# Darioxavierl/OFDM-LTE

Measured on AMD Instinct MI355X. Metric: LTE subframes/sec (20 MHz, 64-QAM, Rayleigh+turbo) at 1/2/4/8 GPU; BER match, higher is better.
Workload: dtype f64

## Files before the change

ofdm-lte_amd/csrc/lte_turbo.hip:

```cpp
#include "lte_common.h"
#include "lte_internal.h"
#include "lte_dev.h"

namespace lte {


constexpr int DM_CH = 64;
#ifndef LTE_DM_NT
#define LTE_DM_NT 0
#endif
template <class R>
__device__ __forceinline__ void dm_store(R* dst, R v, bool add) {
  if (add) *dst = *dst + (R)0.5 * v;
  else if (LTE_DM_NT & 1) __builtin_nontemporal_store((R)0.5 * ((R)0 + v), dst);
  else *dst = (R)0.5 * ((R)0 + v);
}

template <class R>
__global__ __launch_bounds__(256) void k_dematch(const R* __restrict__ llr, int T, int B,
                                                 const int32_t* __restrict__ rx_map, int add,
                                                 R* const* __restrict__ blk, const int64_t* __restrict__ rows,
                                                 int ch, int g0) {
  __shared__ R tile[64][DM_CH + 1];
  const int g = g0 + blockIdx.y;
  const int t0 = blockIdx.x * DM_CH;
  const int nt = min(DM_CH, T - t0);
  const int c4 = (threadIdx.x & 15) * 4;
  for (int f = threadIdx.x >> 4; f < 64; f += 16) {
    const int b = g * 64 + f;
    const R* src = llr + (size_t)b * T + t0;
    R v[4] = {(R)0, (R)0, (R)0, (R)0};
    if (b < B) {
#pragma unroll
      for (int e = 0; e < 4; ++e)
        if (c4 + e < nt) v[e] = src[c4 + e];
    }
#pragma unroll
    for (int e = 0; e < 4; ++e) tile[f][c4 + e] = v[e];
  }
  __syncthreads();
  const int wv = __builtin_amdgcn_readfirstlane(threadIdx.x >> 6), f = threadIdx.x & 63;
  for (int c = wv; c < nt; c += 4) {
    const int m = rx_map[t0 + c];
    if (m < 0) continue;
    const int r = m >> 24, row = m & 0xFFFFFF;
    dm_store(&blk[r][turbo_elem_ch(ch, rows[r], g, row) + f], tile[f][c], add != 0);
  }
}

template <class R>
int launch_dematch(hipStream_t s, const R* llr, int T, int B, const int32_t* rx_map, int n_layers, R* const* blk,
                   const int64_t* rows, int ch, int g0, int add0) {
  const int G = (B + 63) / 64 - g0;
  if (G < 1 || G > 65535 || n_layers < 1) return (int)hipErrorInvalidValue;
  for (int k = 0; k < n_layers; ++k) {
    hipLaunchKernelGGL(k_dematch<R>, dim3((T + DM_CH - 1) / DM_CH, G), dim3(256), 0, s, llr, T, B,
                       rx_map + (size_t)k * T, k > 0 || add0 ? 1 : 0, blk, rows, ch, g0);
    const int e = (int)hipGetLastError();
    if (e) return e;
  }
  return 0;
}

#ifndef LTE_DZ_RE64
#define LTE_DZ_RE64 8
#endif
template <class R> constexpr int dz_re() { return sizeof(R) == 8 ? LTE_DZ_RE64 : 16; }
template <class R, int BPS>
__global__ __launch_bounds__(256) void k_dematch_zn(const cx<R>* __restrict__ z, const R* __restrict__ nv, int n_re,
                                                    int nd, int n_nv, int nv_grp, int nv_sh, int B,
                                                    const int32_t* __restrict__ rx_map, int add,
                                                    R* const* __restrict__ blk, const int64_t* __restrict__ rows,
                                                    int ch, int g0) {
  using V = cx<R>;
  constexpr int DZ_RE = dz_re<R>(), TC = DZ_RE * BPS, PER = 64 * DZ_RE / 256;
  __shared__ R tile[64][TC + 1];
  const int g = g0 + blockIdx.y;
  const int re0 = blockIdx.x * DZ_RE;
  const int nr = min(DZ_RE, n_re - re0);
  V zv[PER];
  R nvv[PER];
#pragma unroll
  for (int k = 0; k < PER; ++k) {
    const int e = threadIdx.x + k * 256, f = e / DZ_RE, r = e % DZ_RE, b = g * 64 + f;
    const bool ok = b < B && r < nr;
    const size_t i = (size_t)b * n_re + re0 + r;
    const int l = (re0 + r) / nd, j = re0 + r - l * nd;
    if (LTE_DM_NT & 2) {
      zv[k] = ok ? mkc(__builtin_nontemporal_load(&z[i].x), __builtin_nontemporal_load(&z[i].y)) : mkc((R)0, (R)0);
      nvv[k] = ok ? __builtin_nontemporal_load(&nv[(size_t)b * n_nv + (l / nv_grp) * (nd >> nv_sh) + (j >> nv_sh)])
                  : (R)1;
    } else {
      zv[k] = ok ? z[i] : mkc((R)0, (R)0);
      nvv[k] = ok ? nv[(size_t)b * n_nv + (l / nv_grp) * (nd >> nv_sh) + (j >> nv_sh)] : (R)1;
    }
  }
#pragma unroll
  for (int k = 0; k < PER; ++k) {
    const int e = threadIdx.x + k * 256, f = e / DZ_RE, r = e % DZ_RE;
    R o[BPS];
    soft_demap<BPS>(zv[k], nvv[k], o);
#pragma unroll
    for (int m = 0; m < BPS; ++m) tile[f][r * BPS + m] = o[m];
  }
  __syncthreads();
  const int t0 = re0 * BPS, nt = nr * BPS;
  const int wv = __builtin_amdgcn_readfirstlane(threadIdx.x >> 6), f = threadIdx.x & 63;
  for (int c = wv; c < nt; c += 4) {
    const int m = rx_map[t0 + c];
    if (m < 0) continue;
    const int r = m >> 24, row = m & 0xFFFFFF;
    dm_store(&blk[r][turbo_elem_ch(ch, rows[r], g, row) + f], tile[f][c], add != 0);
  }
}

template <class R>
int launch_dematch_zn(hipStream_t s, const cx<R>* z, const R* nv, int n_re, int nd, int bps, int B,
                      const int32_t* rx_map, int n_layers, R* const* blk, const int64_t* rows, int ch, int g0,
                      int nv_pairs, int add0) {
  const int G = (B + 63) / 64 - g0;
  if (G < 1 || G > 65535 || (bps != 4 && bps != 6) || n_layers < 1 || nd < 1) return (int)hipErrorInvalidValue;
  if (nv_pairs && (nd & 1)) return (int)hipErrorInvalidValue;
  const int nv_grp = nv_pairs ? 1 : 14, nv_sh = nv_pairs ? 1 : 0;
  const int n_nv = ((n_re / nd + nv_grp - 1) / nv_grp) * (nd >> nv_sh);
  constexpr int DZ = dz_re<R>();
  const dim3 grid((n_re + DZ - 1) / DZ, G);
  const int T = n_re * bps;
  for (int k = 0; k < n_layers; ++k) {
    const int32_t* mp = rx_map + (size_t)k * T;
    if (bps == 4)
      hipLaunchKernelGGL((k_dematch_zn<R, 4>), grid, dim3(256), 0, s, z, nv, n_re, nd, n_nv, nv_grp, nv_sh, B, mp,
                         k > 0 || add0 ? 1 : 0, blk, rows, ch, g0);
    else
      hipLaunchKernelGGL((k_dematch_zn<R, 6>), grid, dim3(256), 0, s, z, nv, n_re, nd, n_nv, nv_grp, nv_sh, B, mp,
                         k > 0 || add0 ? 1 : 0, blk, rows, ch, g0);
    const int e = (int)hipGetLastError();
    if (e) return e;
  }
  return 0;
}

template int launch_dematch<float>(hipStream_t, const float*, int, int, const int32_t*, int, float* const*,
                                   const int64_t*, int, int, int);
template int launch_dematch<double>(hipStream_t, const double*, int, int, const int32_t*, int, double* const*,
                                    const int64_t*, int, int, int);
template int launch_dematch_zn<float>(hipStream_t, const float2*, const float*, int, int, int, int, const int32_t*,
                                      int, float* const*, const int64_t*, int, int, int, int);
template int launch_dematch_zn<double>(hipStream_t, const double2*, const double*, int, int, int, int,
                                       const int32_t*, int, double* const*, const int64_t*, int, int, int, int);


template <class R>
__global__ __launch_bounds__(256) void k_harq_zero(const int32_t* __restrict__ zmap, int nz,
                                                   R* const* __restrict__ blk, const int64_t* __restrict__ rows,
                                                   int ch) {
  const int i = blockIdx.x * 4 + __builtin_amdgcn_readfirstlane(threadIdx.x >> 6);
  if (i >= nz) return;
  const int m = zmap[i], r = m >> 24, row = m & 0xFFFFFF;
  blk[r][turbo_elem_ch(ch, rows[r], blockIdx.y, row) + (threadIdx.x & 63)] = (R)0;
}

template <class R>
int launch_harq_zero(hipStream_t s, const int32_t* zmap, int nz, int G, R* const* blk, const int64_t* rows, int ch) {
  if (nz < 1 || G < 1 || G > 65535) return (int)hipErrorInvalidValue;
  hipLaunchKernelGGL(k_harq_zero<R>, dim3((nz + 3) / 4, G), dim3(256), 0, s, zmap, nz, blk, rows, ch);
  return (int)hipGetLastError();
}
template int launch_harq_zero<float>(hipStream_t, const int32_t*, int, int, float* const*, const int64_t*, int);
template int launch_harq_zero<double>(hipStream_t, const int32_t*, int, int, double* const*, const int64_t*, int);

__global__ __launch_bounds__(64) void k_harq_latch(int B, int t, uint32_t* __restrict__ frame_err,
                                                   uint32_t* __restrict__ frame_crc, uint32_t* __restrict__ tx_used,
                                                   uint32_t* __restrict__ l_err, uint32_t* __restrict__ l_crc,
                                                   uint32_t* __restrict__ skip) {
  const int g = blockIdx.x, b = g * 64 + (int)threadIdx.x;
  bool active = false;
  if (b < B) {
    if (t == 0 || !l_crc[b]) {
      const uint32_t e = frame_err[b], c = frame_crc[b];
      tx_used[b] = (uint32_t)(t + 1);
      l_err[b] = e;
      l_crc[b] = c;
      active = c == 0;
    } else {
      frame_err[b] = l_err[b];
      frame_crc[b] = l_crc[b];
    }
  }
  const unsigned long long still = __ballot(active);
  if (threadIdx.x == 0) skip[g] = still == 0ull ? 1u : 0u;
}

int launch_harq_latch(hipStream_t s, int B, int t, uint32_t* frame_err, uint32_t* frame_crc, uint32_t* tx_used,
                      uint32_t* l_err, uint32_t* l_crc, uint32_t* skip) {
  if (B < 1 || t < 0) return (int)hipErrorInvalidValue;
  hipLaunchKernelGGL(k_harq_latch, dim3((B + 63) / 64), dim3(64), 0, s, B, t, frame_err, frame_crc, tx_used, l_err,
                     l_crc, skip);
  return (int)hipGetLastError();
}

__global__ __launch_bounds__(256) void k_rate_dematch(const double* __restrict__ llr, int E, int Ncb, int n_out,
                                                      const int32_t* __restrict__ src0, int64_t ncb,
                                                      double* __restrict__ out) {
  const int64_t t = (int64_t)blockIdx.x * 256 + threadIdx.x;
  if (t >= ncb * n_out) return;
  const int64_t c = t / n_out;
  const int j = (int)(t - c * n_out);
  double v = 0.0;
  const double* l = llr + c * E;
  for (int i = src0[j]; i >= 0 && i < E; i += Ncb) v = v + l[i];
  out[t] = v;
}

int launch_rate_dematch(hipStream_t s, const double* llr, int E, int Ncb, int n_out, const int32_t* src0, int64_t ncb,
                        double* out) {
  const int64_t n = ncb * n_out;
  if (n <= 0) return 0;
  hipLaunchKernelGGL(k_rate_dematch, dim3((unsigned)((n + 255) / 256)), dim3(256), 0, s, llr, E, Ncb, n_out, src0, ncb,
                     out);
  return (int)hipGetLastError();
}

struct BitWriter {
  uint32_t* p;
  uint64_t acc;
  int n;
  __device__ __forceinline__ void put(uint32_t bits, int nb) {
    acc = (acc << nb) | (nb == 32 ? (uint64_t)bits : (uint64_t)(bits & ((1u << nb) - 1u)));
    n += nb;
    if (n >= 32) {
      *p++ = (uint32_t)(acc >> (n - 32));
      n -= 32;
    }
  }
  __device__ __forceinline__ void flush() {
    if (n) *p = (uint32_t)(acc << (32 - n));
  }
};


__device__ __forceinline__ uint32_t rsc_word(uint32_t u, int nb, uint32_t& s0, uint32_t& s1, uint32_t& s2,
                                             uint32_t* fw) {
  uint32_t y = u ^ (u >> 2) ^ (u >> 3) ^ (u >> 4);
  y ^= y >> 7;
  y ^= y >> 14;
  y ^= y >> 28;
  const uint32_t a = y ^ (s0 ? 0x72e5cb97u : 0u) ^ (s1 ? 0xe5cb972eu : 0u) ^ (s2 ? 0xb972e5cbu : 0u);
  const uint32_t q = a ^ ((a >> 1) | (s0 << 31)) ^ ((a >> 3) | (s2 << 31) | (s1 << 30) | (s0 << 29));
  s0 = (a >> (32 - nb)) & 1u;
  s1 = (a >> (33 - nb)) & 1u;
  s2 = (a >> (34 - nb)) & 1u;
  *fw = a;
  return q;
}

__device__ __forceinline__ uint32_t rsc_tail(uint32_t& s0, uint32_t& s1, uint32_t& s2) {
  const uint32_t fb = 0u, par = fb ^ s0 ^ s2;
  s2 = s1; s1 = s0; s0 = fb;
  return fb | (par << 1);
}

constexpr int ENC_SEG = 4;
constexpr int ENC_MAXSW = 48;
constexpr int ENC_CH = 16;

struct X2Tab { uint32_t v[16]; };
constexpr X2Tab make_x2tab(uint32_t poly) {
  X2Tab t{};
  uint32_t b = 2u;
  for (int j = 0; j < 16; ++j) {
    t.v[j] = b;
    uint32_t r = 0u;
    for (int i = 23; i >= 0; --i) {
      r = ((r << 1) & 0xFFFFFFu) ^ ((r & 0x800000u) ? poly : 0u);
      r ^= ((b >> i) & 1u) ? b : 0u;
    }
    b = r;
  }
  return t;
}
__constant__ X2Tab kX2B = make_x2tab((uint32_t)CRC24B_POLY);

__device__ __forceinline__ uint32_t crcb_xpow(int e) {
  uint32_t r = 1u;
  for (int j = 0; j < 16; ++j)
    if ((e >> j) & 1) r = gf24_mul(r, kX2B.v[j], (uint32_t)CRC24B_POLY);
  return r;
}

__device__ __forceinline__ uint32_t rsc_zero_steps(uint32_t st, int n) {
  uint32_t s0 = st & 1u, s1 = (st >> 1) & 1u, s2 = (st >> 2) & 1u;
  for (int k = n % 7; k > 0; --k) {
    const uint32_t fb = s1 ^ s2;
    s2 = s1; s1 = s0; s0 = fb;
  }
  return s0 | (s1 << 1) | (s2 << 2);
}

__device__ __forceinline__ uint32_t rsc_seg_start(const uint32_t* fin, int q, int lane, int K, int SW) {
  uint32_t st = 0u;
  for (int p = 0; p < q; ++p) {
    const int len = max(0, min(K, 32 * (p + 1) * SW) - 32 * p * SW);
    st = rsc_zero_steps(st, len) ^ fin[p * 64 + lane];
  }
  return st;
}

__global__ __launch_bounds__(64 * ENC_SEG) void k_encode(const uint32_t* __restrict__ pw, int PW, int KWmax,
                                                         uint32_t* __restrict__ enc, int EW,
                                                         const CbInfo* __restrict__ cbi, int B,
                                                         const uint16_t* __restrict__ qmask, int qstride) {
  extern __shared__ uint32_t esm[];
  uint32_t* cwl = esm;
  uint32_t* xch = esm + (size_t)KWmax * 64;
  __shared__ uint32_t crc_t[256];
  for (int i = threadIdx.x; i < 256; i += blockDim.x) crc_t[i] = crc24_table_entry(i, (uint32_t)CRC24B_POLY);
  const int G = (B + 63) >> 6;
  const int r = blockIdx.x / G;
  const int lane = threadIdx.x & 63, q = __builtin_amdgcn_readfirstlane(threadIdx.x >> 6);
  const int b = (blockIdx.x - r * G) * 64 + lane;
  const bool act = b < B;
  const CbInfo ci = cbi[r];
  const int K = ci.K, F = ci.F, C = gridDim.x / G;
  const int KW = (K + 31) >> 5, KWf = K >> 5;
  const int SW = (KW + ENC_SEG - 1) / ENC_SEG;
  const int w0 = min(KW, q * SW), w1 = min(KW, w0 + SW);
  const bool last = w0 < w1 && w1 == KW;
  const uint32_t* tb = pw + (size_t)(act ? b : 0) * PW;
  uint32_t* e = enc + ((size_t)(act ? b : 0) * C + r) * 3 * EW;
  const int Kd = ci.crc ? K - 24 : K;
  const int64_t base = (int64_t)ci.off - F;
  const int64_t i00 = base >> 5;
  const int o = (int)(base & 31);
  auto ldw = [&](int64_t i) -> uint32_t { return (i >= 0 && i < PW) ? tb[i] : 0u; };
  __syncthreads();
  uint32_t crc = 0u;
  {
    uint32_t wa = ldw(i00 + w0), wb = ldw(i00 + w0 + 1);
    for (int w = w0; w < w1; ++w) {
      const uint32_t wn = ldw(i00 + w + 2);
      const int p0 = w * 32;
      uint32_t t = o ? ((wa << o) | (wb >> (32 - o))) : wa;
      if (p0 < F) t &= (F - p0 >= 32) ? 0u : (0xFFFFFFFFu >> (F - p0));
      const int db = min(32, max(0, Kd - p0));
      t &= db >= 32 ? 0xFFFFFFFFu : ~(0xFFFFFFFFu >> db);
      if (ci.crc)
#pragma unroll
        for (int k = 0; k < 4; ++k)
          if (8 * k < db) crc = ((crc << 8) & 0xFFFFFFu) ^ crc_t[((crc >> 16) ^ (t >> (24 - 8 * k))) & 0xFFu];
      cwl[w * 64 + lane] = t;
      wa = wb;
      wb = wn;
    }
  }
  xch[q * 64 + lane] = (ci.crc && 32 * w0 < Kd)
                           ? gf24_mul(crc, crcb_xpow(Kd - min(32 * w1, Kd)), (uint32_t)CRC24B_POLY) : 0u;
  __syncthreads();
  if (ci.crc) {
    crc = 0u;
#pragma unroll
    for (int p = 0; p < ENC_SEG; ++p) crc ^= xch[p * 64 + lane];
    const uint32_t L = crc << 8;
    for (int w = max(w0, Kd >> 5); w < w1; ++w) {
      const int p0 = 32 * w;
      cwl[w * 64 + lane] |= p0 <= Kd ? (L >> (Kd - p0)) : (L << (p0 - Kd));
    }
  }
  uint32_t s0 = 0u, s1 = 0u, s2 = 0u, f;
  uint32_t F2 = 0u;
  const uint16_t* qm = qmask + (size_t)r * qstride;
  for (int w = w0; w < w1; ++w) {
    const uint32_t cwv = cwl[w * 64 + lane];
    const int nb = min(32, K - 32 * w);
    (void)rsc_word(cwv, nb, s0, s1, s2, &f);
    const uint32_t* qw = reinterpret_cast<const uint32_t*>(qm + 32 * w);
#pragma unroll
    for (int j = 0; j < 32; j += 2) {
      const uint32_t pr = qw[j >> 1];
      F2 ^= (pr & 0xFFFFu) & (0u - ((cwv >> (31 - j)) & 1u));
      F2 ^= (pr >> 16) & (0u - ((cwv >> (30 - j)) & 1u));
    }
  }
  xch[(ENC_SEG + q) * 64 + lane] = s0 | (s1 << 1) | (s2 << 2);
  xch[(2 * ENC_SEG + q) * 64 + lane] = F2;
  __syncthreads();
  uint32_t st = rsc_seg_start(xch + ENC_SEG * 64, q, lane, K, SW);
  s0 = st & 1u; s1 = (st >> 1) & 1u; s2 = (st >> 2) & 1u;
  uint32_t pf = 0, pq = 0;
  int pnb = 0;
  for (int wc = w0; wc < w1; wc += ENC_CH) {
    uint32_t fb[ENC_CH], qb[ENC_CH];
#pragma unroll
    for (int j = 0; j < ENC_CH; ++j) {
      const int w = wc + j;
      fb[j] = qb[j] = 0u;
      if (w >= w1) continue;
      const int nb = min(32, K - 32 * w);
      const uint32_t qq = rsc_word(cwl[w * 64 + lane], nb, s0, s1, s2, &f);
      if (nb == 32) { fb[j] = f; qb[j] = qq; }
      else { pf = f; pq = qq; pnb = nb; }
    }
    if (act) {
#pragma unroll
      for (int j = 0; j < ENC_CH; ++j)
        if (wc + j < min(w1, KWf)) e[wc + j] = fb[j];
#pragma unroll
      for (int j = 0; j < ENC_CH; ++j)
        if (wc + j < min(w1, KWf)) e[EW + wc + j] = qb[j];
    }
  }
  if (last && act) {
    BitWriter wr0{e + KWf, 0, 0}, wr1{e + EW + KWf, 0, 0};
    if (pnb) {
      wr0.put(pf >> (32 - pnb), pnb);
      wr1.put(pq >> (32 - pnb), pnb);
    }
    for (int t = 0; t < 3; ++t) {
      const uint32_t v = rsc_tail(s0, s1, s2);
      wr0.put(v & 1u, 1);
      wr1.put(v >> 1, 1);
    }
    wr0.flush();
    wr1.flush();
  }
  {
    uint32_t fall = 0u;
#pragma unroll
    for (int p = 0; p < ENC_SEG; ++p) fall ^= xch[(2 * ENC_SEG + p) * 64 + lane];
    uint32_t st2 = 0u;
    for (int t = 0; t < q; ++t) {
      const int len = max(0, min(K, 32 * (t + 1) * SW) - 32 * t * SW);
      st2 = rsc_zero_steps(st2, len) ^ ((fall >> (3 * t)) & 7u);
    }
    s0 = st2 & 1u; s1 = (st2 >> 1) & 1u; s2 = (st2 >> 2) & 1u;
  }
  pq = 0;
  pnb = 0;
  {
    const int k0 = 32 * w0;
    int pi0 = (int)(((int64_t)ci.f1 * k0 + (int64_t)ci.f2 * k0 % K * k0) % K);
    int d0 = (int)(((int64_t)ci.f1 + (int64_t)ci.f2 * (2 * (int64_t)k0 + 1)) % K);
    const float invK = 1.0f / (float)K;
    const int f2l = (int)(((int64_t)ci.f2 * lane * (lane - 1)) % K);
    const char* cwb = reinterpret_cast<const char*>(cwl) + 4 * lane;
    for (int w = w0; w < w1; w += 2) {
      int x = pi0 + (int)((lane * (int64_t)d0) % K) + f2l;
      x -= (int)((float)x * invK) * K;
      x += x < 0 ? K : 0;
      x -= x >= K ? K : 0;
      const int rowb = (x >> 5) << 8, shf = x & 31;
      uint32_t qw[2] = {0u, 0u};
#pragma unroll
      for (int h = 0; h < 2; ++h) {
        if (w + h >= w1) break;
        const int nb = min(32, K - 32 * (w + h));
        uint32_t u = 0u;
#pragma unroll
        for (int j = 0; j < 32; ++j) {
          const int a = __builtin_amdgcn_readlane(rowb, 32 * h + j);
          const int sh = __builtin_amdgcn_readlane(shf, 32 * h + j);
          const uint32_t v = *reinterpret_cast<const uint32_t*>(cwb + a);
          u |= ((v << sh) >> 31) << (31 - j);
        }
        const uint32_t qq = rsc_word(u, nb, s0, s1, s2, &f);
        if (nb == 32) qw[h] = qq;
        else { pq = qq; pnb = nb; }
      }
      if (act) {
        if (w < KWf) e[2 * EW + w] = qw[0];
        if (w + 1 < min(w1, KWf)) e[2 * EW + w + 1] = qw[1];
      }
      pi0 = (int)(((int64_t)pi0 + 64 * (int64_t)d0 + (int64_t)ci.f2 * 64 * 63) % K);
      d0 = (int)(((int64_t)d0 + 128 * (int64_t)ci.f2) % K);
    }
  }
  if (last && act) {
    BitWriter wr2{e + 2 * EW + KWf, 0, 0};
    if (pnb) wr2.put(pq >> (32 - pnb), pnb);
    for (int t = 0; t < 3; ++t) {
      const uint32_t v = rsc_tail(s0, s1, s2);
      const int pos = K + 3 + t;
      if (v & 1u) e[pos >> 5] |= 1u << (31 - (pos & 31));
      wr2.put(v >> 1, 1);
    }
    wr2.flush();
  }
}

void encode_qmask(const CbInfo* cbs, int C, int qstride, uint16_t* out) {
  std::fill(out, out + (size_t)C * qstride, (uint16_t)0);
  for (int r = 0; r < C; ++r) {
    const int K = cbs[r].K, KW = (K + 31) / 32, SW = (KW + ENC_SEG - 1) / ENC_SEG;
    uint16_t v[7];
    uint32_t st = 1u;
    for (int m = 0; m < 7; ++m) {
      v[m] = (uint16_t)st;
      const uint32_t s0 = st & 1u, s1 = (st >> 1) & 1u, s2 = (st >> 2) & 1u;
      st = (s1 ^ s2) | (s0 << 1) | (s1 << 2);
    }
    for (int64_t k = 0; k < K; ++k) {
      const int p = (int)((cbs[r].f1 * k + (int64_t)cbs[r].f2 * k % K * k) % K);
      const int t = (int)(k / (32 * SW)), end = std::min(32 * SW * (t + 1), K);
      out[(size_t)r * qstride + p] = (uint16_t)(v[(end - 1 - k) % 7] << (3 * t));
    }
  }
}

int launch_encode(hipStream_t s, const uint32_t* pw, int PW, int KWmax, uint32_t* enc, int EW,
                  const CbInfo* cbi_dev, int C, int B, const uint16_t* qmask, int qstride) {
  const int64_t blocks = (int64_t)C * ((B + 63) / 64);
  const size_t shm = ((size_t)KWmax * 64 + 3 * ENC_SEG * 64) * sizeof(uint32_t);
  if (blocks > 0x7FFFFFFF || KWmax > 4 * ENC_MAXSW + 1 || shm > 65536 || !qmask) return (int)hipErrorInvalidValue;
  hipLaunchKernelGGL(k_encode, dim3((unsigned)blocks), dim3(64 * ENC_SEG), shm, s, pw, PW, KWmax, enc, EW, cbi_dev,
                     B, qmask, qstride);
  return (int)hipGetLastError();
}


__device__ __forceinline__ uint32_t get32s(const uint32_t* w, int64_t st, int64_t p, int64_t nwords) {
  const int64_t i = p >> 5;
  const int o = (int)(p & 31);
  const uint32_t a = w[i * st];
  if (o == 0) return a;
  const uint32_t b = (i + 1 < nwords) ? w[(i + 1) * st] : 0u;
  return (a << o) | (b >> (32 - o));
}

constexpr int CRC_SEG = 8;
constexpr int CRC_MAXC = 32;
struct CrcSeg { uint32_t x[CRC_SEG]; };

__global__ __launch_bounds__(64 * CRC_SEG) void k_crc_count(const CbInfo* __restrict__ cbi, int C,
                                                            uint32_t* const* __restrict__ dec,
                                                            const int* __restrict__ KW, int B,
                                                            const uint32_t* __restrict__ pw, int PW, int n_bits,
                                                            int SW, CrcSeg xs, uint32_t* __restrict__ frame_err,
                                                            uint32_t* __restrict__ frame_crc,
                                                            uint8_t* __restrict__ cap_bits, int b0,
                                                            const uint64_t* __restrict__ fid, uint64_t seed) {
  __shared__ uint32_t T[1024];
  __shared__ uint32_t part[3][CRC_SEG][64];
  __shared__ int s_off[CRC_MAXC], s_end[CRC_MAXC], s_F[CRC_MAXC], s_kw[CRC_MAXC];
  __shared__ const uint32_t* s_dec[CRC_MAXC];
  crc24_slice4_fill(T, (uint32_t)CRC24A_POLY);
  if (threadIdx.x < C) {
    const CbInfo ci = cbi[threadIdx.x];
    s_off[threadIdx.x] = ci.off;
    s_end[threadIdx.x] = ci.off + ci.info;
    s_F[threadIdx.x] = ci.F;
    s_kw[threadIdx.x] = KW[threadIdx.x];
    s_dec[threadIdx.x] = dec[threadIdx.x];
  }
  __syncthreads();
  const int lane = threadIdx.x & 63, seg = __builtin_amdgcn_readfirstlane(threadIdx.x >> 6);
  const int b = b0 + blockIdx.x * 64 + lane;
  const bool act = b < B;
  const int bb = act ? b : b0;
  const int g = bb >> 6, gl = bb & 63;
  const uint32_t* tx = pw + (size_t)bb * PW;
  const uint64_t fr = fid ? fid[bb] : 0ull;
  u32x4 rv{0u, 0u, 0u, 0u};
  int rvg = -1;
  const int Btb = n_bits + 24;
  const int nw = (Btb + 31) >> 5;
  const int w0 = seg * SW, w1 = min(nw, w0 + SW);
  uint32_t crc = 0, err = 0, rx_crc = 0;
  int r = 0, off = s_off[0], end = s_end[0], F = s_F[0], kw = s_kw[0];
  const uint32_t* base = s_dec[0] + (size_t)g * kw * 64 + gl;
  for (int w = w0; w < w1; ++w) {
    uint32_t word = 0;
    int got = 0;
    const int want = min(32, Btb - 32 * w);
    while (got < want) {
      const int j = 32 * w + got;
      while (j >= end) {
        ++r;
        off = s_off[r]; end = s_end[r]; F = s_F[r]; kw = s_kw[r];
        base = s_dec[r] + (size_t)g * kw * 64 + gl;
      }
      const int avail = min(want - got, end - j);
      const uint32_t v = get32s(base, 64, (int64_t)F + (j - off), kw);
      const uint32_t m = avail >= 32 ? 0xFFFFFFFFu : ~(0xFFFFFFFFu >> avail);
      word |= (v & m) >> got;
      got += avail;
    }
    const int dbits = min(32, max(0, n_bits - 32 * w));
    if (dbits == 32) {
      crc = crc24_slice4(T, crc, word);
    } else {
      int k = 0;
      for (; k + 8 <= dbits; k += 8) {
        const uint32_t byte = (word >> (24 - k)) & 0xFFu;
        crc = ((crc << 8) & 0xFFFFFFu) ^ T[((crc >> 16) ^ byte) & 0xFFu];
      }
      for (; k < dbits; ++k) {
        const uint32_t bit = (word >> (31 - k)) & 1u;
        const uint32_t msb = (crc >> 23) & 1u;
        crc = (crc << 1) & 0xFFFFFFu;
        if (msb ^ bit) crc ^= (uint32_t)CRC24A_POLY;
      }
      for (int q = max(0, n_bits - 32 * w); q < want; ++q)
        rx_crc |= ((word >> (31 - q)) & 1u) << (23 - (32 * w + q - n_bits));
    }
    if (dbits > 0) {
      const uint32_t m = dbits >= 32 ? 0xFFFFFFFFu : ~(0xFFFFFFFFu >> dbits);
      uint32_t t;
      if (fid) {
        if ((w >> 2) != rvg) {
          rvg = w >> 2;
          rv = rng4(seed, fr, RNG_STREAM_BITS, (uint32_t)rvg);
        }
        t = (w & 3) == 0 ? rv.x : (w & 3) == 1 ? rv.y : (w & 3) == 2 ? rv.z : rv.w;
      } else {
        t = tx[w];
      }
      err += __popc((word ^ t) & m);
    }
    if (cap_bits && act) {
      for (int q = 0; q < dbits; ++q) cap_bits[(size_t)b * n_bits + 32 * w + q] = (word >> (31 - q)) & 1u;
    }
  }
  part[0][seg][lane] = gf24_mul(crc, xs.x[seg], (uint32_t)CRC24A_POLY);
  part[1][seg][lane] = err;
  part[2][seg][lane] = rx_crc;
  __syncthreads();
  if (seg == 0 && act) {
    uint32_t c = 0, e = 0, rc = 0;
#pragma unroll
    for (int s2 = 0; s2 < CRC_SEG; ++s2) {
      c ^= part[0][s2][lane];
      e += part[1][s2][lane];
      rc |= part[2][s2][lane];
    }
    frame_err[b] = e;
    frame_crc[b] = (c == rc) ? 1u : 0u;
  }
}

int launch_crc_count(hipStream_t s, const CbInfo* cbi_dev, int C, uint32_t* const* dec, const int* KW, int B,
                     const uint32_t* pw, int PW, int n_bits, uint32_t* frame_err, uint32_t* frame_crc,
                     uint8_t* cap_bits, int b0, const uint64_t* fid, uint64_t seed) {
  if (b0 < 0 || b0 >= B || n_bits < 0 || C < 1 || C > CRC_MAXC) return (int)hipErrorInvalidValue;
  const int nw = (n_bits + 24 + 31) >> 5;
  const int SW = (nw + CRC_SEG - 1) / CRC_SEG;
  CrcSeg xs{};
  for (int sg = 0; sg < CRC_SEG; ++sg) {
    const int end = std::min(32 * (sg + 1) * SW, n_bits);
    xs.x[sg] = gf24_xpow((uint64_t)(n_bits - std::max(end, 0)), (uint32_t)CRC24A_POLY);
  }
  hipLaunchKernelGGL(k_crc_count, dim3((B - b0 + 63) / 64), dim3(64 * CRC_SEG), 0, s, cbi_dev, C, dec, KW, B, pw, PW,
                     n_bits, SW, xs, frame_err, frame_crc, cap_bits, b0, fid, seed);
  return (int)hipGetLastError();
}

}
```

Measured before the change: 180,000.

## Restructure dematch_zn to loop over OFDM symbols with prefetch and grouped blocks

Replaces the per-RE-tile soft-demap and dematch kernel with one whose blocks own a subcarrier chunk and loop over all symbols. The next symbol's z, noise-variance, map and row pointers are prefetched while the current tile is written out. Destination addresses are computed once per tile column and broadcast with readlane, and the add/store path and channel count become template parameters. Block indices are grouped by 64-row batches to improve locality. This cuts launch-grid size, repeated index maths and load latency, at the cost of a serial symbol loop per block, fewer blocks, and higher register use.

```diff
diff --git a/ofdm-lte_amd/csrc/lte_turbo.hip b/ofdm-lte_amd/csrc/lte_turbo.hip
--- a/ofdm-lte_amd/csrc/lte_turbo.hip
+++ b/ofdm-lte_amd/csrc/lte_turbo.hip
@@ -66,6 +66,10 @@
 #define LTE_DZ_RE64 8
 #endif
 template <class R> constexpr int dz_re() { return sizeof(R) == 8 ? LTE_DZ_RE64 : 16; }
+#ifndef LTE_DZ_ORDER
+#define LTE_DZ_ORDER 2
+#endif
+#if LTE_DZ_ORDER == 0
 template <class R, int BPS>
 __global__ __launch_bounds__(256) void k_dematch_zn(const cx<R>* __restrict__ z, const R* __restrict__ nv, int n_re,
                                                     int nd, int n_nv, int nv_grp, int nv_sh, int B,
@@ -139,6 +143,158 @@
   }
   return 0;
 }
+#else
+constexpr int DZ_GW = LTE_DZ_ORDER == 2 ? 8 : 32;
+
+template <class R, bool ADD>
+__device__ __forceinline__ void dz_store(__attribute__((address_space(1))) R* dst, R old, R v) {
+  if (ADD) *dst = old + (R)0.5 * v;
+  else if (LTE_DM_NT & 1) __builtin_nontemporal_store((R)0.5 * ((R)0 + v), dst);
+  else *dst = (R)0.5 * ((R)0 + v);
+}
+
+template <class R, int BPS, int CH, bool ADD>
+__global__ __launch_bounds__(256) void k_dematch_zn(const cx<R>* __restrict__ z, const R* __restrict__ nv, int n_sym,
+                                                    int nd, int n_nv, int nv_grp, int nv_sh, int B,
+                                                    const int32_t* __restrict__ rx_map, R* const* __restrict__ blk,
+                                                    const int64_t* __restrict__ rows, int G, int g0) {
+  using V = cx<R>;
+  using GP = __attribute__((address_space(1))) R*;
+  constexpr int DZ_RE = dz_re<R>(), TC = DZ_RE * BPS, PER = 64 * DZ_RE / 256, NI = TC / 4;
+  static_assert(TC % 4 == 0 && NI <= 64, "one lane per tile column of a wave");
+  __shared__ R tile[64][TC + 1];
+  const int nj = (nd + DZ_RE - 1) / DZ_RE;
+  const int q = blockIdx.x / (DZ_GW * nj), id = blockIdx.x - q * DZ_GW * nj, w = min(DZ_GW, G - q * DZ_GW);
+  const int g = g0 + q * DZ_GW + id % w, j0 = (id / w) * DZ_RE;
+  const int nr = min(DZ_RE, nd - j0), nt = nr * BPS, n_re = n_sym * nd;
+  const int wv = __builtin_amdgcn_readfirstlane(threadIdx.x >> 6), lane = threadIdx.x & 63;
+  const int c = wv + 4 * lane;
+  const bool mok = lane < NI && c < nt;
+  const int32_t* mp = rx_map + (size_t)j0 * BPS + c;
+  auto ld_map = [&](int l) -> int { return mok && l < n_sym ? mp[(size_t)l * nd * BPS] : -1; };
+  int m1 = ld_map(0), m2 = ld_map(1);
+  size_t zi[PER], ni[PER];
+  bool ok[PER];
+#pragma unroll
+  for (int k = 0; k < PER; ++k) {
+    const int e = threadIdx.x + k * 256, f = e / DZ_RE, r = e % DZ_RE, b = g * 64 + f;
+    ok[k] = b < B && r < nr;
+    zi[k] = (size_t)b * n_re + j0 + r;
+    ni[k] = (size_t)b * n_nv + ((j0 + r) >> nv_sh);
+  }
+  V zv[PER];
+  R nvv[PER];
+  auto ld_z = [&](int l) {
+#pragma unroll
+    for (int k = 0; k < PER; ++k) {
+      const size_t i = zi[k] + (size_t)l * nd;
+      if (LTE_DM_NT & 2)
+        zv[k] = ok[k] ? mkc(__builtin_nontemporal_load(&z[i].x), __builtin_nontemporal_load(&z[i].y))
+                      : mkc((R)0, (R)0);
+      else
+        zv[k] = ok[k] ? z[i] : mkc((R)0, (R)0);
+    }
+  };
+  auto ld_nv = [&](int l) {
+#pragma unroll
+    for (int k = 0; k < PER; ++k) {
+      const size_t i = ni[k] + (size_t)(l / nv_grp) * (nd >> nv_sh);
+      if (LTE_DM_NT & 2) nvv[k] = ok[k] ? __builtin_nontemporal_load(&nv[i]) : (R)1;
+      else nvv[k] = ok[k] ? nv[i] : (R)1;
+    }
+  };
+  R* rb = nullptr;
+  int64_t rr = 0;
+  auto ld_row = [&]() {
+    if (m1 >= 0) {
+      rb = blk[m1 >> 24];
+      rr = rows[m1 >> 24];
+    }
+  };
+  ld_z(0);
+  ld_nv(0);
+  ld_row();
+  for (int l = 0; l < n_sym; ++l) {
+    const uint64_t dst = m1 >= 0 ? (uint64_t)(rb + turbo_elem<CH>(rr, g, m1 & 0xFFFFFF)) : 0;
+#pragma unroll
+    for (int k = 0; k < PER; ++k) {
+      const int e = threadIdx.x + k * 256, f = e / DZ_RE, r = e % DZ_RE;
+      R o[BPS];
+      soft_demap<BPS>(zv[k], nvv[k], o);
+#pragma unroll
+      for (int m = 0; m < BPS; ++m) tile[f][r * BPS + m] = o[m];
+    }
+    __syncthreads();
+    m1 = m2;
+    if (l + 1 < n_sym) {
+      ld_z(l + 1);
+      if ((l + 1) % nv_grp == 0) ld_nv(l + 1);
+      ld_row();
+      m2 = ld_map(l + 2);
+    }
+    R v[NI], old[NI];
+    GP d[NI];
+#pragma unroll
+    for (int i = 0; i < NI; ++i) {
+      v[i] = tile[lane][wv + 4 * i];
+      const uint32_t lo = __builtin_amdgcn_readlane((int)(uint32_t)dst, i);
+      const uint32_t hi = __builtin_amdgcn_readlane((int)(uint32_t)(dst >> 32), i);
+      d[i] = (GP)(((uint64_t)hi << 32) | lo);
+    }
+    if (ADD) {
+#pragma unroll
+      for (int i = 0; i < NI; ++i) old[i] = d[i] ? d[i][lane] : (R)0;
+    }
+#pragma unroll
+    for (int i = 0; i < NI; ++i)
+      if (d[i]) dz_store<R, ADD>(d[i] + lane, old[i], v[i]);
+    __syncthreads();
+  }
+}
+
+template <class R, int BPS, int CH>
+static void dz_launch(hipStream_t s, int nblk, const cx<R>* z, const R* nv, int n_sym, int nd, int n_nv, int nv_grp,
+                      int nv_sh, int B, const int32_t* mp, bool add, R* const* blk, const int64_t* rows, int G,
+                      int g0) {
+  if (add)
+    hipLaunchKernelGGL((k_dematch_zn<R, BPS, CH, true>), dim3(nblk), dim3(256), 0, s, z, nv, n_sym, nd, n_nv, nv_grp,
+                       nv_sh, B, mp, blk, rows, G, g0);
+  else
+    hipLaunchKernelGGL((k_dematch_zn<R, BPS, CH, false>), dim3(nblk), dim3(256), 0, s, z, nv, n_sym, nd, n_nv, nv_grp,
+                       nv_sh, B, mp, blk, rows, G, g0);
+}
+
+template <class R>
+int launch_dematch_zn(hipStream_t s, const cx<R>* z, const R* nv, int n_re, int nd, int bps, int B,
+                      const int32_t* rx_map, int n_layers, R* const* blk, const int64_t* rows, int ch, int g0,
+                      int nv_pairs, int add0) {
+  const int G = (B + 63) / 64 - g0;
+  if (G < 1 || G > 65535 || (bps != 4 && bps != 6) || n_layers < 1 || nd < 1) return (int)hipErrorInvalidValue;
+  if (nv_pairs && (nd & 1)) return (int)hipErrorInvalidValue;
+  if (n_re < nd || n_re % nd || (ch != 1 && ch != TURBO_CH)) return (int)hipErrorInvalidValue;
+  const int nv_grp = nv_pairs ? 1 : 14, nv_sh = nv_pairs ? 1 : 0;
+  const int n_sym = n_re / nd;
+  const int n_nv = ((n_sym + nv_grp - 1) / nv_grp) * (nd >> nv_sh);
+  constexpr int DZ = dz_re<R>();
+  const int64_t nblk = (int64_t)G * ((nd + DZ - 1) / DZ);
+  if (nblk > 0x7FFFFFFF) return (int)hipErrorInvalidValue;
+  const int T = n_re * bps;
+  for (int k = 0; k < n_layers; ++k) {
+    const int32_t* mp = rx_map + (size_t)k * T;
+    const bool add = k > 0 || add0;
+    auto go = [&](auto launch) {
+      launch(s, (int)nblk, z, nv, n_sym, nd, n_nv, nv_grp, nv_sh, B, mp, add, blk, rows, G, g0);
+    };
+    if (bps == 4 && ch == 1) go(dz_launch<R, 4, 1>);
+    else if (bps == 4) go(dz_launch<R, 4, TURBO_CH>);
+    else if (ch == 1) go(dz_launch<R, 6, 1>);
+    else go(dz_launch<R, 6, TURBO_CH>);
+    const int e = (int)hipGetLastError();
+    if (e) return e;
+  }
+  return 0;
+}
+#endif
 
 template int launch_dematch<float>(hipStream_t, const float*, int, int, const int32_t*, int, float* const*,
                                    const int64_t*, int, int, int);
```

Result: no change. 180,000 (-0.0%).
